# haoy945/DeMF

Hardware: AMD Instinct MI355X
Metric: DeMF fusion fwd+bwd scenes/sec at 20k pts + 530x730 RGB (higher is better)
Workload: dtype f32; 1 GPU; BASELINE configs[2]: full DeMF fusion hot path fwd+loss+bwd+allreduce+AdamW, 8 scenes/GPU x (20000 pts, 800x1120 -> 4-level 256-ch pyramid), 256 queries, H=8 L=4 P=2, fp32; compute_mode=f32, scenes_per_gpu=8, parallelism=dp1, cloud=uniform

## Files before the change

demf_amd/csrc/mlp.hip:

```cpp
#include "mlp_dev.h"
#include <type_traits>

namespace demf {

#ifdef DEMF_MLP_PROFILE
__device__ long long g_mlp_prof[16];
#define MP_T(k) const long long mp##k = __builtin_readcyclecounter();
#define MP_ACC(i, a, b) if (mp_on) mp_acc[i] += (b) - (a);
#else
#define MP_T(k)
#define MP_ACC(i, a, b)
#endif

template <int NT, int RT, int PRO, bool STATS, bool POOL = false, bool FIRST = false, bool RED = false,
          int CM = 0, bool SEL = false>
__global__ __launch_bounds__(256, 2) void mlp_gemm_kernel(MlpArgs p) {
  static_assert(!SEL || POOL, "SEL is a mode of the pooled epilogue");
  static_assert(!(STATS && RED) && !(FIRST && RED), "one column-sum epilogue at a time");
  constexpr bool BF16 = CM == 1, X3 = CM == 2;
  constexpr int LDB = X3 ? MLP_LD3 : MLP_LD;
  constexpr int WROWS = 32 * RT;
  constexpr int BROWS = 4 * WROWS;
  constexpr int NVEC = PRO == PRO_NONE ? 0 : (PRO == PRO_BNRELU ? 2 : 5);
  __shared__ __attribute__((aligned(16))) float s_a[4][WROWS * MLP_LD];
  __shared__ __attribute__((aligned(16))) float s_b[NT * 32 * LDB];
  __shared__ __attribute__((aligned(16))) float s_vec[NVEC ? NVEC * MLP_MAXK : 4];
  __shared__ float s_red[(STATS || RED) ? 4 * NT * 32 * 2 : (FIRST ? 4 * NT * 32 * 10 + 16 : 1)];
  __shared__ float4 s_pool[(POOL && RT == 1) ? 4 * NT * 32 : 1];
  if constexpr (NVEC > 0) {
    for (int i = threadIdx.x; i < NVEC * p.K; i += 256) s_vec[i] = p.vec[i];
    __syncthreads();
  }
  const int lane = threadIdx.x & 63;
  const int wave = threadIdx.x >> 6;
  const int lr = lane & 31, lh = lane >> 5;
  float* sa = s_a[wave];
  int bx = blockIdx.x, gx = gridDim.x, by = blockIdx.y;
  if constexpr (POOL) {
    if (p.halves == 2) {
      by = (bx >> 3) & 1;
      bx = (bx & 7) | ((bx >> 4) << 3);
      gx >>= 1;
    }
  }
  const int cofs = by * NT * 32;
  const int ntiles = (p.R + BROWS - 1) / BROWS;
  const int ksteps = (p.K + MLP_BK - 1) / MLP_BK;
  __shared__ int s_next;
  const bool dyn = p.sched != nullptr;
  const int grp = (bx >> 3) & (SCHED_GROUPS - 1);
  const int grp_first = gx / SCHED_GROUPS;
  auto group_tile = [&](int j) { return (((j >> 3) * SCHED_GROUPS + grp) << 3) + (j & 7); };
  int claimed = 0;
  float cs1[NT], cs2[NT];
#pragma unroll
  for (int nt = 0; nt < NT; ++nt) cs1[nt] = cs2[nt] = 0.f;
  float fs[FIRST ? NT : 1][10];
  float4 fcx = make_float4(0.f, 0.f, 0.f, 0.f);
  if constexpr (FIRST) {
#pragma unroll
    for (int nt = 0; nt < NT; ++nt)
#pragma unroll
      for (int q = 0; q < 10; ++q) fs[nt][q] = 0.f;
  }
  f32x16 acc[RT][NT];
  unsigned selbits = 0;
  if constexpr (SEL) {
#pragma unroll
    for (int nt = 0; nt < NT; ++nt) {
      const int col = cofs + nt * 32 + lr;
      if (col < p.N && p.fin.gamma[col] < 0.f) selbits |= 1u << nt;
    }
  }

  const int pr = lane >> 3, pc = (lane & 7) * 4;
  const int br = threadIdx.x >> 3;
  MlpRaw<PRO> pre[4 * RT];
  bool pok[4 * RT];
  float4 preb[NT];
  auto prefetch = [&](int tile, int ks) {
    const int k0 = ks * MLP_BK;
    const int row0 = tile * BROWS + wave * WROWS;
#pragma unroll
    for (int it = 0; it < 4 * RT; ++it) {
      const int row = row0 + it * 8 + pr, col = k0 + pc;
      pok[it] = row < p.R && col < p.K;
      mlp_fetch<PRO>(p, row, col, pok[it], pre[it]);
    }
#pragma unroll
    for (int i = 0; i < NT; ++i) {
      const int n = cofs + br + 32 * i, col = k0 + pc;
      preb[i] = make_float4(0.f, 0.f, 0.f, 0.f);
      if (p.ldb > 0) {
        const int kk = k0 + br, nn = cofs + 32 * i + pc;
        if (kk < p.K && nn < p.N) preb[i] = *reinterpret_cast<const float4*>(p.Bt + (size_t)kk * p.ldb + nn);
      } else if (n < p.N && col < p.K) {
        preb[i] = *reinterpret_cast<const float4*>(p.Bt + (size_t)n * p.K + col);
      }
    }
  };
#ifdef DEMF_MLP_PROFILE
  long long mp_acc[8] = {0, 0, 0, 0, 0, 0, 0, 0};
  const bool mp_on = blockIdx.x == 0 && blockIdx.y == 0 && threadIdx.x == 0;
#endif
  int tile = bx;
  if (tile < ntiles) prefetch(tile, 0);

  int ks = 0;
  while (tile < ntiles) {
    MP_T(0)
    const int k0 = ks * MLP_BK;
    const int row0 = tile * BROWS + wave * WROWS;
    const bool last_ks = ks == ksteps - 1;
    if (dyn && threadIdx.x == 0) {
      if (ks == 0) claimed = group_tile(grp_first + atomicAdd(p.sched + grp, 1));
      if (last_ks) s_next = claimed;
    }
    float* sb = s_b;
    if (ks == 0) {
#pragma unroll
      for (int rt = 0; rt < RT; ++rt)
#pragma unroll
        for (int nt = 0; nt < NT; ++nt)
#pragma unroll
          for (int r = 0; r < 16; ++r) acc[rt][nt][r] = 0.f;
    }
    lds_barrier();
    MP_T(1) MP_ACC(0, mp0, mp1)
    if constexpr (BF16) {
      char* sab = reinterpret_cast<char*>(sa);
      char* sbb = reinterpret_cast<char*>(sb);
#pragma unroll
      for (int it = 0; it < 4 * RT; ++it)
        *reinterpret_cast<bf16x4*>(sab + (it * 8 + pr) * (4 * MLP_LD) + 2 * pc) =
            to_bf16x4(mlp_xform<PRO>(p, s_vec, k0 + pc, pok[it], pre[it]));
#pragma unroll
      for (int i = 0; i < NT; ++i)
        if (p.ldb > 0) {
          char* d = sbb + (32 * i + pc) * (4 * MLP_LD) + 2 * br;
          *reinterpret_cast<__bf16*>(d) = (__bf16)preb[i].x;
          *reinterpret_cast<__bf16*>(d + 4 * MLP_LD) = (__bf16)preb[i].y;
          *reinterpret_cast<__bf16*>(d + 8 * MLP_LD) = (__bf16)preb[i].z;
          *reinterpret_cast<__bf16*>(d + 12 * MLP_LD) = (__bf16)preb[i].w;
        } else {
          *reinterpret_cast<bf16x4*>(sbb + (br + 32 * i) * (4 * MLP_LD) + 2 * pc) = to_bf16x4(preb[i]);
        }
    } else if constexpr (X3) {
#pragma unroll
      for (int it = 0; it < 4 * RT; ++it)
        *reinterpret_cast<float4*>(sa + (it * 8 + pr) * MLP_LD + pc) =
            mlp_xform<PRO>(p, s_vec, k0 + pc, pok[it], pre[it]);
      char* sbb = reinterpret_cast<char*>(sb);
#pragma unroll
      for (int i = 0; i < NT; ++i) {
        bf16x4 h, m, l;
        split3(preb[i], h, m, l);
        if (p.ldb > 0) {
#pragma unroll
          for (int e = 0; e < 4; ++e) {
            char* d = sbb + (32 * i + pc + e) * (4 * MLP_LD3) + 2 * br;
            *reinterpret_cast<__bf16*>(d) = h[e];
            *reinterpret_cast<__bf16*>(d + 64) = m[e];
            *reinterpret_cast<__bf16*>(d + 128) = l[e];
          }
        } else {
          char* d = sbb + (br + 32 * i) * (4 * MLP_LD3) + 2 * pc;
          *reinterpret_cast<bf16x4*>(d) = h;
          *reinterpret_cast<bf16x4*>(d + 64) = m;
          *reinterpret_cast<bf16x4*>(d + 128) = l;
        }
      }
    } else {
#pragma unroll
    for (int it = 0; it < 4 * RT; ++it)
      *reinterpret_cast<float4*>(sa + (it * 8 + pr) * MLP_LD + pc) =
          mlp_xform<PRO>(p, s_vec, k0 + pc, pok[it], pre[it]);
#pragma unroll
    for (int i = 0; i < NT; ++i)
      if (p.ldb > 0) {
        float* d = sb + (32 * i + pc) * MLP_LD + br;
        d[0] = preb[i].x; d[MLP_LD] = preb[i].y; d[2 * MLP_LD] = preb[i].z; d[3 * MLP_LD] = preb[i].w;
      } else {
        *reinterpret_cast<float4*>(sb + (br + 32 * i) * MLP_LD + pc) = preb[i];
      }
    }
    MP_T(2) MP_ACC(1, mp1, mp2)
    lds_barrier();
    MP_T(3) MP_ACC(2, mp2, mp3)
    constexpr bool DEFER = (POOL && RT == 2) || FIRST;
    const bool defer_prefetch = DEFER && last_ks;
    const int next_tile = last_ks ? (dyn ? s_next : tile + gx) : tile;
    const int next_ks = last_ks ? 0 : ks + 1;
    if (next_tile < ntiles && !defer_prefetch) prefetch(next_tile, next_ks);
    MP_T(4) MP_ACC(3, mp3, mp4)
    float4 yq[(FIRST || RED) ? 2 * RT * 2 : 1];
    float4 xq = make_float4(0.f, 0.f, 0.f, 0.f);
    auto first_load = [&](int half) {
#pragma unroll
      for (int j = 0; j < 2 * RT * 2; ++j) {
        const int id = lane + 64 * j;
        const int row = row0 + (id >> 3);
        yq[j] = make_float4(0.f, 0.f, 0.f, 0.f);
        if (row < p.R && cofs + 32 * half + 4 * (id & 7) < p.N)
          yq[j] = *reinterpret_cast<const float4*>(p.fY + (size_t)row * p.fld + p.fc0 + cofs + 32 * half + 4 * (id & 7));
      }
    };
    auto first_store = [&]() {
#pragma unroll
      for (int j = 0; j < 2 * RT * 2; ++j) {
        const int id = lane + 64 * j;
        *reinterpret_cast<float4*>(sa + (id >> 3) * MLP_LD + 4 * (id & 7)) = yq[j];
      }
    };
    if constexpr (RED) {
      if (last_ks) first_load(0);
    }
    if constexpr (FIRST) {
      if (last_ks) {
        first_load(0);
        if (lane < WROWS && row0 + lane < p.R)
          xq = *reinterpret_cast<const float4*>(p.fX + (size_t)(row0 + lane) * 4);
      }
    }
    if constexpr (BF16) {
      const char* sab = reinterpret_cast<const char*>(sa);
      const char* sbb = reinterpret_cast<const char*>(sb);
      const int kch = min(MLP_BK / 16, (p.K - k0 + 15) / 16);
      for (int c16 = 0; c16 < kch; ++c16) {
        bf16x8 a8[RT];
#pragma unroll
        for (int rt = 0; rt < RT; ++rt)
          a8[rt] = *reinterpret_cast<const bf16x8*>(sab + (rt * 32 + lr) * (4 * MLP_LD) + 2 * (c16 * 16 + 8 * lh));
#pragma unroll
        for (int nt = 0; nt < NT; ++nt) {
          const bf16x8 b8 = *reinterpret_cast<const bf16x8*>(sbb + (nt * 32 + lr) * (4 * MLP_LD) + 2 * (c16 * 16 + 8 * lh));
#pragma unroll
          for (int rt = 0; rt < RT; ++rt)
            acc[rt][nt] = __builtin_amdgcn_mfma_f32_32x32x16_bf16(a8[rt], b8, acc[rt][nt], 0, 0, 0);
        }
      }
    } else if constexpr (X3) {
      const char* sbb = reinterpret_cast<const char*>(sb);
      const int kch = min(MLP_BK / 16, (p.K - k0 + 15) / 16);
      for (int c16 = 0; c16 < kch; ++c16) {
        bf16x8 ah[RT], am[RT], al[RT];
#pragma unroll
        for (int rt = 0; rt < RT; ++rt) {
          const float* src = sa + (rt * 32 + lr) * MLP_LD + c16 * 16 + 8 * lh;
          split3(*reinterpret_cast<const float4*>(src), *reinterpret_cast<const float4*>(src + 4),
                 ah[rt], am[rt], al[rt]);
        }
#pragma unroll
        for (int nt = 0; nt < NT; ++nt) {
          const char* src = sbb + (nt * 32 + lr) * (4 * MLP_LD3) + 2 * (c16 * 16 + 8 * lh);
          const bf16x8 bh = *reinterpret_cast<const bf16x8*>(src);
          const bf16x8 bm = *reinterpret_cast<const bf16x8*>(src + 64);
          const bf16x8 bl = *reinterpret_cast<const bf16x8*>(src + 128);
#pragma unroll
          for (int rt = 0; rt < RT; ++rt) {
            acc[rt][nt] = __builtin_amdgcn_mfma_f32_32x32x16_bf16(al[rt], bh, acc[rt][nt], 0, 0, 0);
            acc[rt][nt] = __builtin_amdgcn_mfma_f32_32x32x16_bf16(ah[rt], bl, acc[rt][nt], 0, 0, 0);
            acc[rt][nt] = __builtin_amdgcn_mfma_f32_32x32x16_bf16(am[rt], bm, acc[rt][nt], 0, 0, 0);
            acc[rt][nt] = __builtin_amdgcn_mfma_f32_32x32x16_bf16(am[rt], bh, acc[rt][nt], 0, 0, 0);
            acc[rt][nt] = __builtin_amdgcn_mfma_f32_32x32x16_bf16(ah[rt], bm, acc[rt][nt], 0, 0, 0);
            acc[rt][nt] = __builtin_amdgcn_mfma_f32_32x32x16_bf16(ah[rt], bh, acc[rt][nt], 0, 0, 0);
          }
        }
      }
    } else {
    const int kchunks = min(MLP_BK / 8, (p.K - k0 + 7) / 8);
    for (int c8 = 0; c8 < kchunks; ++c8) {
      float4 a4[RT];
#pragma unroll
      for (int rt = 0; rt < RT; ++rt)
        a4[rt] = *reinterpret_cast<const float4*>(sa + (rt * 32 + lr) * MLP_LD + c8 * 8 + 4 * lh);
#pragma unroll
      for (int nt = 0; nt < NT; ++nt) {
        const float4 b4 = *reinterpret_cast<const float4*>(sb + (nt * 32 + lr) * MLP_LD + c8 * 8 + 4 * lh);
#pragma unroll
        for (int rt = 0; rt < RT; ++rt) {
          acc[rt][nt] = __builtin_amdgcn_mfma_f32_32x32x2f32(a4[rt].x, b4.x, acc[rt][nt], 0, 0, 0);
          acc[rt][nt] = __builtin_amdgcn_mfma_f32_32x32x2f32(a4[rt].y, b4.y, acc[rt][nt], 0, 0, 0);
          acc[rt][nt] = __builtin_amdgcn_mfma_f32_32x32x2f32(a4[rt].z, b4.z, acc[rt][nt], 0, 0, 0);
          acc[rt][nt] = __builtin_amdgcn_mfma_f32_32x32x2f32(a4[rt].w, b4.w, acc[rt][nt], 0, 0, 0);
        }
      }
    }
    }
    MP_T(5) MP_ACC(4, mp4, mp5)
    if (last_ks) {
#pragma unroll
      for (int nt = 0; nt < NT; ++nt) {
        float s1 = 0.f, s2 = 0.f;
        if constexpr (FIRST) {
          const int col = cofs + nt * 32 + lr;
          const bool cok = col < p.N;
          const float sc0 = cok ? p.fss[p.fc0 + col] : 0.f, sh0 = cok ? p.fss[p.fld + p.fc0 + col] : 0.f;
          const float mu0 = cok ? p.fmi[p.fc0 + col] : 0.f, is0 = cok ? p.fmi[p.fld + p.fc0 + col] : 0.f;
          first_store();
          if (nt == 0 && lane < WROWS) *reinterpret_cast<float4*>(sa + lane * MLP_LD + MLP_BK) = xq;
          if (nt + 1 < NT) first_load(nt + 1);
#pragma unroll
          for (int rt = 0; rt < RT; ++rt)
#pragma unroll
            for (int r = 0; r < 16; ++r) {
              const int rl = rt * 32 + (r & 3) + 8 * (r >> 2) + 4 * lh;
              if ((r & 3) == 0) __builtin_amdgcn_sched_barrier(0);
              if (row0 + rl < p.R && cok) {
                const float y = sa[rl * MLP_LD + lr];
                const float4 x = *reinterpret_cast<const float4*>(sa + rl * MLP_LD + MLP_BK);
                const float dz = __builtin_fmaf(y, sc0, sh0) > 0.f ? acc[rt][nt][r] : 0.f;
                fs[nt][0] += dz;
                fs[nt][1] = __builtin_fmaf(dz, (y - mu0) * is0, fs[nt][1]);
                fs[nt][2] = __builtin_fmaf(dz, x.x, fs[nt][2]);
                fs[nt][3] = __builtin_fmaf(dz, x.y, fs[nt][3]);
                fs[nt][4] = __builtin_fmaf(dz, x.z, fs[nt][4]);
                fs[nt][5] = __builtin_fmaf(dz, x.w, fs[nt][5]);
                fs[nt][6] = __builtin_fmaf(y, x.x, fs[nt][6]);
                fs[nt][7] = __builtin_fmaf(y, x.y, fs[nt][7]);
                fs[nt][8] = __builtin_fmaf(y, x.z, fs[nt][8]);
                fs[nt][9] = __builtin_fmaf(y, x.w, fs[nt][9]);
                if (nt == 0 && lr == 0 && by == 0) { fcx.x += x.x; fcx.y += x.y; fcx.z += x.z; fcx.w += x.w; }
              }
            }
        } else {
        float sc0 = 0.f, sh0 = 0.f, mu0 = 0.f, is0 = 0.f;
        if constexpr (RED) {
          const int col = cofs + nt * 32 + lr;
          if (col < p.N) {
            sc0 = p.fss[p.fc0 + col]; sh0 = p.fss[p.fld + p.fc0 + col];
            mu0 = p.fmi[p.fc0 + col]; is0 = p.fmi[p.fld + p.fc0 + col];
          }
          first_store();
          if (nt + 1 < NT) first_load(nt + 1);
        }
        auto store_tile = [&](auto full_c) {
          constexpr bool FULL = decltype(full_c)::value;
#pragma unroll
          for (int rt = 0; rt < RT; ++rt)
#pragma unroll
            for (int r = 0; r < 16; ++r) {
              const int row = row0 + rt * 32 + (r & 3) + 8 * (r >> 2) + 4 * lh;
              const float v = acc[rt][nt][r];
              const bool ok = FULL || (row < p.R && cofs + nt * 32 + lr < p.N);
              if (ok) p.Y[(size_t)row * p.ldy + cofs + nt * 32 + lr] = v;
              if constexpr (RED) {
                if ((r & 3) == 0) __builtin_amdgcn_sched_barrier(0);
                if (ok) {
                  const float y = sa[(rt * 32 + (r & 3) + 8 * (r >> 2) + 4 * lh) * MLP_LD + lr];
                  const float dz = __builtin_fmaf(y, sc0, sh0) > 0.f ? v : 0.f;
                  s1 += dz;
                  s2 = __builtin_fmaf(dz, (y - mu0) * is0, s2);
                }
              }
            }
          if constexpr (STATS) {
            using f32x2 = float __attribute__((ext_vector_type(2)));
            f32x2 a1 = {0.f, 0.f}, a2 = {0.f, 0.f};
#pragma unroll
            for (int rt = 0; rt < RT; ++rt)
#pragma unroll
              for (int r = 0; r < 16; r += 2) {
                const f32x2 v = {acc[rt][nt][r], acc[rt][nt][r + 1]};
                a1 += v;
                a2 = __builtin_elementwise_fma(v, v, a2);
              }
            s1 += a1.x + a1.y;
            s2 += a2.x + a2.y;
          }
        };
        if constexpr (POOL) {
          if (tile * BROWS + BROWS <= p.R && cofs + NT * 32 <= p.N) store_tile(std::true_type{});
          else store_tile(std::false_type{});
        } else {
#pragma unroll
          for (int rt = 0; rt < RT; ++rt)
#pragma unroll
            for (int r = 0; r < 16; ++r) {
              const int row = row0 + rt * 32 + (r & 3) + 8 * (r >> 2) + 4 * lh;
              const float v = acc[rt][nt][r];
              if (row < p.R && cofs + nt * 32 + lr < p.N)
                p.Y[(size_t)row * p.ldy + cofs + nt * 32 + lr] = v;
              if constexpr (RED) {
                if ((r & 3) == 0) __builtin_amdgcn_sched_barrier(0);
                if (row < p.R && cofs + nt * 32 + lr < p.N) {
                  const float y = sa[(rt * 32 + (r & 3) + 8 * (r >> 2) + 4 * lh) * MLP_LD + lr];
                  const float dz = __builtin_fmaf(y, sc0, sh0) > 0.f ? v : 0.f;
                  s1 += dz;
                  s2 = __builtin_fmaf(dz, (y - mu0) * is0, s2);
                }
              }
              if constexpr (STATS) {
                s1 += v;
                s2 = __builtin_fmaf(v, v, s2);
              }
            }
        }
        }
        cs1[nt] += s1;
        cs2[nt] += s2;
        if constexpr (POOL) {
          {
            const int col = cofs + nt * 32 + lr;
            if constexpr (SEL) {
              const unsigned flip = ((selbits >> nt) & 1u) << 31;
              if (p.ns == 16) pool_epilogue_sel<RT, NT, 16>(p, acc, nt, row0, col, lh, flip);
              else if (p.ns == 32) pool_epilogue_sel<RT, NT, 32>(p, acc, nt, row0, col, lh, flip);
              else if constexpr (RT == 2) pool_epilogue_sel<RT, NT, 64>(p, acc, nt, row0, col, lh, flip);
              else pool_half_reduce_sel<NT>(acc, nt, wave, lr, lh, s_pool, flip);
            } else {
            if (p.ns == 16) pool_epilogue<RT, NT, 16>(p, acc, nt, row0, col, lh);
            else if (p.ns == 32) pool_epilogue<RT, NT, 32>(p, acc, nt, row0, col, lh);
            else if constexpr (RT == 2) pool_epilogue<RT, NT, 64>(p, acc, nt, row0, col, lh);
            else pool_half_reduce<NT>(acc, nt, wave, lr, lh, s_pool);
            }
          }
        }
      }
      if constexpr (POOL && RT == 1) {
        if (p.ns == 64) {
          lds_barrier();
          if ((wave & 1) == 0 && lh == 0) {
            const int grow = row0;
#pragma unroll
            for (int nt = 0; nt < NT; ++nt) {
              const int col = cofs + nt * 32 + lr;
              if constexpr (SEL) {
                const float2* sp = reinterpret_cast<const float2*>(s_pool);
                const float2 a = sp[(wave * NT + nt) * 32 + lr];
                const float2 b = sp[((wave + 1) * NT + nt) * 32 + lr];
                const bool take_b = b.x > a.x;
                if (grow < p.R && col < p.N) {
                  const unsigned flip = ((selbits >> nt) & 1u) << 31;
                  const size_t o = (size_t)(grow / 64) * p.N + col;
                  p.pmax[o] = flip_sign(take_b ? b.x : a.x, flip);
                  p.amax[o] = __builtin_bit_cast(int, take_b ? b.y : a.y);
                }
                continue;
              }
              const float4 a = s_pool[(wave * NT + nt) * 32 + lr];
              const float4 b = s_pool[((wave + 1) * NT + nt) * 32 + lr];
              float mx = a.x, mn = a.y;
              int ax = __builtin_bit_cast(int, a.z), an = __builtin_bit_cast(int, a.w);
              if (b.x > mx) { mx = b.x; ax = __builtin_bit_cast(int, b.z); }
              if (b.y < mn) { mn = b.y; an = __builtin_bit_cast(int, b.w); }
              if (grow < p.R && col < p.N) {
                const size_t o = (size_t)(grow / 64) * p.N + col;
                p.pmax[o] = mx; p.pmin[o] = mn; p.amax[o] = ax; p.amin[o] = an;
              }
            }
          }
        }
      }
      if constexpr ((POOL && RT == 2) || FIRST) {
        if (next_tile < ntiles) prefetch(next_tile, next_ks);
      }
    }
    MP_T(6) MP_ACC(5, mp5, mp6)
    tile = next_tile;
    ks = next_ks;
  }
#ifdef DEMF_MLP_PROFILE
  if (mp_on) { for (int i = 0; i < 8; ++i) atomicAdd((unsigned long long*)&g_mlp_prof[i], (unsigned long long)mp_acc[i]); atomicAdd((unsigned long long*)&g_mlp_prof[15], 1ull); }
#endif
  if (dyn) {
    if (threadIdx.x == 0) {
      int* gdone = p.sched + SCHED_GROUPS;
      const int members = (int)(gridDim.x * gridDim.y) / SCHED_GROUPS;
      if (atomicAdd(gdone + 1 + grp, 1) == members - 1) {
        atomicExch(gdone + 1 + grp, 0);
        atomicExch(p.sched + grp, 0);
        if (atomicAdd(gdone, 1) == SCHED_GROUPS - 1) atomicExch(gdone, 0);
      }
    }
  }
  if constexpr (FIRST) {
#pragma unroll
    for (int nt = 0; nt < NT; ++nt)
#pragma unroll
      for (int q = 0; q < 10; ++q) {
        const float v = fs[nt][q] + __shfl_xor(fs[nt][q], 32);
        if (lh == 0) s_red[((wave * NT + nt) * 10 + q) * 32 + lr] = v;
      }
    fcx.x += __shfl_xor(fcx.x, 32); fcx.y += __shfl_xor(fcx.y, 32);
    fcx.z += __shfl_xor(fcx.z, 32); fcx.w += __shfl_xor(fcx.w, 32);
    if (lane == 0) {
      float* c = s_red + 4 * NT * 32 * 10 + wave * 4;
      c[0] = fcx.x; c[1] = fcx.y; c[2] = fcx.z; c[3] = fcx.w;
    }
    __syncthreads();
    constexpr int PER = NT * 10 * 32;
    for (int i = threadIdx.x; i < PER; i += 256) {
      const float v = s_red[i] + s_red[PER + i] + s_red[2 * PER + i] + s_red[3 * PER + i];
      const int nt = i / 320, q = (i / 32) % 10, c = i & 31;
      const int col = cofs + nt * 32 + c;
      if (col < p.N) {
        const int dst = q < 2 ? q * p.N + col : (q < 6 ? 2 * p.N + col * 4 + (q - 2) : 6 * p.N + col * 4 + (q - 6));
        atomicAdd(p.fsum + dst, (double)v);
      }
    }
    if (threadIdx.x < 4 && by == 0) {
      const float* c = s_red + 4 * NT * 32 * 10;
      atomicAdd(p.fsum + 10 * p.N + threadIdx.x,
                (double)(c[threadIdx.x] + c[4 + threadIdx.x] + c[8 + threadIdx.x] + c[12 + threadIdx.x]));
    }
  }
  if constexpr (STATS || RED) {
#pragma unroll
    for (int nt = 0; nt < NT; ++nt) {
      cs1[nt] += __shfl_xor(cs1[nt], 32);
      cs2[nt] += __shfl_xor(cs2[nt], 32);
      if (lh == 0) {
        s_red[(wave * NT + nt) * 64 + lr] = cs1[nt];
        s_red[(wave * NT + nt) * 64 + 32 + lr] = cs2[nt];
      }
    }
    __syncthreads();
    const int lin_s = (int)(blockIdx.y * gridDim.x + blockIdx.x);
    double* sdst = p.stats;
    if constexpr (RED) {
      if (p.vfin.ticket != nullptr && p.vfin.racc != nullptr) sdst = repl_copy(p.vfin.racc, p.fld, lin_s);
    } else {
      if (p.fin.ss != nullptr && p.fin.racc != nullptr) sdst = repl_copy(p.fin.racc, p.N, lin_s);
    }
    for (int i = threadIdx.x; i < NT * 64; i += 256) {
      const float v = s_red[i] + s_red[NT * 64 + i] + s_red[2 * NT * 64 + i] + s_red[3 * NT * 64 + i];
      const int nt = i >> 6, which = (i >> 5) & 1, c = i & 31;
      if (cofs + nt * 32 + c < p.N)
        atomicAdd(sdst + which * (RED ? p.fld : p.N) + (RED ? p.fc0 : 0) + cofs + nt * 32 + c, (double)v);
    }
  }
  if constexpr (RED) {
    if (p.vfin.ticket != nullptr) {
      sync_drained();
      if (threadIdx.x == 0)
        s_next = last_workgroup(p.vfin.ticket, (int)(gridDim.x * gridDim.y), (int)(blockIdx.y * gridDim.x + blockIdx.x));
      __syncthreads();
      if (s_next) bn_vec_finalize(p.vfin, p.fld, p.fc0, p.N, p.stats, threadIdx.x, 256);
    }
  }
  if constexpr (STATS) {
    if (p.fin.ss != nullptr) {
      sync_drained();
      if (threadIdx.x == 0) {
        const int total = (int)(gridDim.x * gridDim.y);
        const int lin = (int)(blockIdx.y * gridDim.x + blockIdx.x);
        const int ngroups = total < SCHED_GROUPS ? total : SCHED_GROUPS;
        const int g = lin % SCHED_GROUPS;
        const int members = total / SCHED_GROUPS + (g < total % SCHED_GROUPS ? 1 : 0);
        int* t = p.fin.ticket + FIN_OFF;
        int last = 0;
        asm volatile("s_waitcnt vmcnt(0)" ::: "memory");
        if (atomicAdd(t + 1 + g, 1) == members - 1) {
          atomicExch(t + 1 + g, 0);
          if (atomicAdd(t, 1) == ngroups - 1) { atomicExch(t, 0); last = 1; }
        }
        s_next = last;
      }
      __syncthreads();
      if (s_next) {
        const BnFin& f = p.fin;
        if (threadIdx.x == 0 && f.nbt != nullptr) *f.nbt += 1;
        for (int c = threadIdx.x; c < p.N; c += 256) {
          double s1 = __builtin_bit_cast(
              double, atomicExch(reinterpret_cast<unsigned long long*>(p.stats + c), 0ull));
          double s2 = __builtin_bit_cast(
              double, atomicExch(reinterpret_cast<unsigned long long*>(p.stats + p.N + c), 0ull));
          if (f.racc != nullptr) { s1 += repl_take(f.racc, p.N, c); s2 += repl_take(f.racc, p.N, p.N + c); }
          bn_finalize_channel(c, p.N, f.count, s1, s2, f.gamma, f.beta, f.eps, f.momentum, f.rmean,
                              f.rvar, f.ss, f.mi, f.conv_bias);
        }
      }
    }
  }
}

static int mlp_grid(int R, int brows) {
  const int tiles = (R + brows - 1) / brows;
  const int cap = sw().gemm_grid;
  return tiles < cap ? (tiles > 0 ? tiles : 1) : cap;
}

template <int PRO, bool STATS, bool POOL, bool RED, int CM>
static int launch_gemm_t(const MlpArgs& a, hipStream_t s);

template <int PRO, bool STATS, bool POOL = false, bool RED = false>
static int launch_gemm(const MlpArgs& a, hipStream_t s) {
  switch (compute_mode()) {
    case 1: return launch_gemm_t<PRO, STATS, POOL, RED, 1>(a, s);
    case 2: {
      if (sw().x3_mask & (PRO >= PRO_DY_DENSE ? 2 : 1)) return launch_gemm_t<PRO, STATS, POOL, RED, 2>(a, s);
      return launch_gemm_t<PRO, STATS, POOL, RED, 0>(a, s);
    }
    default: return launch_gemm_t<PRO, STATS, POOL, RED, 0>(a, s);
  }
}

template <int PRO, bool STATS, bool POOL, bool RED, int BF16>
static int launch_gemm_t(const MlpArgs& a, hipStream_t s) {
  if constexpr ((BF16 == 1 || BF16 == 2) && !RED && STATS && PRO == PRO_BNRELU) {
    if (fwd_pc_takes(a, POOL)) {
      const int rc = launch_fwd_pc(a, BF16, POOL, s);
      if (rc == DEMF_OK) set_last_form(DEMF_FORM_PC);
      return rc;
    }
    if (fwd_res_takes(a, POOL)) {
      const int rc = launch_fwd_res(a, BF16, POOL, s);
      if (rc == DEMF_OK) set_last_form(DEMF_FORM_RES);
      return rc;
    }
  }
  if (a.st != 0) {
    set_error("mlp_gemm: bf16 row storage (st=%d) is only built into the weight-resident forward (K = 64, "
              "N = 64 / 128, R >= 16384, bf16 compute mode)", a.st);
    return DEMF_EUNSUPPORTED;
  }
  if constexpr ((BF16 == 1 || BF16 == 2) && !POOL && !STATS && (PRO == PRO_DY_DENSE || PRO == PRO_DY_SPARSE)) {
    constexpr bool SP = PRO == PRO_DY_SPARSE;
    if (dx_tile_takes(a, SP, RED)) {
      const int rc = launch_dx_tile(a, BF16, SP, RED, s);
      if (rc != LAUNCH_TRY_NEXT) { set_last_form(DEMF_FORM_TILE); return rc; }
    }
  }
  if constexpr ((BF16 == 1 || BF16 == 2) && !RED && !POOL && STATS && (PRO == PRO_BNRELU || PRO == PRO_NONE)) {
    if (fwd_tile_takes(a, PRO == PRO_BNRELU)) {
      const int rc = launch_fwd_tile(a, BF16, PRO == PRO_BNRELU, s);
      if (rc != LAUNCH_TRY_NEXT) { set_last_form(DEMF_FORM_TILE); return rc; }
    }
  }
  set_last_form(DEMF_FORM_GENERIC);
  const dim3 block(256);
  constexpr int RT2_MAX = PRO >= PRO_DY_DENSE ? 2 : 4;
  constexpr int NT_MAX = PRO >= PRO_DY_DENSE ? 4 : 8;
  const int nt = (a.N + 31) / 32;
  if (nt < 1 || nt > (POOL ? NT_MAX : 16)) {
    set_error("mlp_gemm: N=%d unsupported for this prologue (max %d columns per launch)", a.N,
              (POOL ? NT_MAX : 16) * 32);
    return DEMF_EUNSUPPORTED;
  }
  if constexpr (POOL) {
    const bool half64 = a.ns == 64 && nt <= 4 && !sw().pool_halves;
    const bool rt2 = a.ns == 64 && !half64;
    const int ntl = rt2 ? (nt < 2 ? nt : 2) : (nt < 4 ? nt : 4);
    const int ys = (nt + ntl - 1) / ntl;
    int gx = mlp_grid(a.R, rt2 ? 256 : 128);
    MlpArgs a2 = a;
    dim3 grid(gx, ys);
    if (ys == 2) {
      gx = ((gx + 7) / 8) * 8;
      a2.halves = 2;
      grid = dim3(2 * gx, 1);
    }
    {
      const int brows = rt2 ? 256 : 128;
      const int tiles = (a.R + brows - 1) / brows;
      if (sw().pool_dyn && ys == 1 && tiles > gx && a.K > MLP_BK && gx % (8 * SCHED_GROUPS) == 0)
        a2.sched = sched_slot();
    }
    const bool sel = a.pmin == nullptr && a.fin.gamma != nullptr;
#define PGO(NTv, RTv)                                                                                       \
    do {                                                                                                    \
      if (sel) hipLaunchKernelGGL((mlp_gemm_kernel<NTv, RTv, PRO, STATS, true, false, false, BF16, true>), grid, block, 0, s, a2); \
      else hipLaunchKernelGGL((mlp_gemm_kernel<NTv, RTv, PRO, STATS, true, false, false, BF16>), grid, block, 0, s, a2);           \
    } while (0)
    if (rt2) { if (ntl == 1) PGO(1, 2); else PGO(2, 2); }
    else if (ntl == 1) PGO(1, 1);
    else if (ntl == 2) PGO(2, 1);
    else if (ntl == 3) PGO(3, 1);
    else PGO(4, 1);
#undef PGO
    return check_launch("mlp_gemm_pool");
  } else {
  const int tiles1 = (a.R + 127) / 128;
  if ((tiles1 < 192 && nt > 1) || nt > NT_MAX || (BF16 == 2 && nt > 4 && sw().x3_wide_split)) {
    int ysplit = (sw().split_target + tiles1 - 1) / tiles1;
    if (ysplit < (nt + 3) / 4) ysplit = (nt + 3) / 4;
    if (ysplit > nt) ysplit = nt;
    const int ntl = (nt + ysplit - 1) / ysplit;
    const dim3 grid(tiles1, (nt + ntl - 1) / ntl);
    switch (ntl) {
#define SPLIT(NTv)                                                                              \
      case NTv: hipLaunchKernelGGL((mlp_gemm_kernel<NTv, 1, PRO, STATS, POOL, false, RED, BF16>), grid, block, 0, s, a); break;
      SPLIT(1) SPLIT(2) SPLIT(3) SPLIT(4)
#undef SPLIT
      default: break;
    }
    if (ntl <= 4) return check_launch("mlp_gemm");
  }
#define GO(NTv, RTv)                                                                            \
  do {                                                                                          \
    MlpArgs a3 = a;                                                                             \
    const int gxv = mlp_grid(a.R, 128 * RTv);                                                   \
    const int tilesv = (a.R + 128 * RTv - 1) / (128 * RTv);                                     \
    if (tilesv > gxv && a.K > MLP_BK && gxv % (8 * SCHED_GROUPS) == 0) a3.sched = sched_slot();                                \
    hipLaunchKernelGGL((mlp_gemm_kernel<NTv, RTv, PRO, STATS, POOL, false, RED, BF16>), dim3(gxv), block, 0, s, a3); \
  } while (0)
#define CASE(NTv)                                                                               \
  case NTv:                                                                                     \
    if constexpr (NTv <= NT_MAX && (BF16 != 2 || NTv <= 4)) {                                   \
      if constexpr (NTv <= RT2_MAX && !RED) GO(NTv, 2); else GO(NTv, 1);                        \
    }                                                                                           \
    break;
  if constexpr (BF16 == 2) {
    if (nt > 4) return launch_gemm_t<PRO, STATS, POOL, RED, 0>(a, s);
  }
  switch (nt) {
    CASE(1) CASE(2) CASE(3) CASE(4) CASE(5) CASE(6) CASE(7) CASE(8)
  }
#undef CASE
#undef GO
  return check_launch("mlp_gemm");
  }
}

static int mlp_check(int R, int K, int N, int ldx) {
  DEMF_REQUIRE(R >= 0 && K >= 4 && K % 4 == 0 && K <= MLP_MAXK && N >= 1 && N <= 256 && ldx >= K &&
                   ldx % 4 == 0,
               "mlp: bad sizes R=%d K=%d N=%d ldx=%d (K%%4==0, K<=512, 1<=N<=256)", R, K, N, ldx);
  return DEMF_OK;
}

}

using namespace demf;


extern "C" int demf_mlp_gemm_fwd(int R, int K, int N, int ldx, const float* X,
                                 const float* pro_scale_shift, const float* Wt, float* Y,
                                 double* stats, demf_stream_t stream) {
  if (int e = mlp_check(R, K, N, ldx)) return e;
  if (R == 0) return DEMF_OK;
  DEMF_REQUIRE(X && Wt && Y, "mlp_gemm_fwd: null pointer");
  MlpArgs a{};
  a.R = R; a.K = K; a.N = N; a.ldx = ldx; a.ldy = N; a.X = X; a.vec = pro_scale_shift; a.Bt = Wt;
  a.Y = Y; a.stats = stats;
  hipStream_t s = (hipStream_t)stream;
  if (pro_scale_shift)
    return stats ? launch_gemm<PRO_BNRELU, true>(a, s) : launch_gemm<PRO_BNRELU, false>(a, s);
  return stats ? launch_gemm<PRO_NONE, true>(a, s) : launch_gemm<PRO_NONE, false>(a, s);
}

extern "C" int demf_mlp_gemm_fwd_pool(int R, int K, int N, int ldx, const float* X,
                                      const float* pro_scale_shift, const float* Wt, float* Y,
                                      double* stats, int ns, float* pmax, float* pmin, int* amax,
                                      int* amin, demf_stream_t stream) {
  if (int e = mlp_check(R, K, N, ldx)) return e;
  const bool ok = (ns == 16 || ns == 32 || ns == 64) && R % ns == 0;
  if (!ok) {
    set_error("mlp_gemm_fwd_pool: ns=%d with R=%d N=%d is not fused", ns, R, N);
    return DEMF_EUNSUPPORTED;
  }
  if (R == 0) return DEMF_OK;
  DEMF_REQUIRE(X && Wt && Y && pro_scale_shift && stats && pmax && pmin && amax && amin,
               "mlp_gemm_fwd_pool: null pointer");
  MlpArgs a{};
  a.R = R; a.K = K; a.N = N; a.ldx = ldx; a.ldy = N; a.X = X; a.vec = pro_scale_shift; a.Bt = Wt;
  a.Y = Y; a.stats = stats; a.ns = ns; a.pmax = pmax; a.pmin = pmin; a.amax = amax; a.amin = amin;
  return launch_gemm<PRO_BNRELU, true, true>(a, (hipStream_t)stream);
}

template <typename Launch>
static int launch_with_finalize(MlpArgs& a, BnFin fin, Launch launch, hipStream_t s) {
  fin.ticket = sw().no_fin ? nullptr : sched_slot();
  fin.racc = fin.ticket != nullptr && a.N <= ACC_MAX_N && sw().acc_repl_fwd ? accum_slot() : nullptr;
  a.fin = fin;
  if (fin.ticket != nullptr) return launch(a);
  a.fin.ss = nullptr;
  if (int e = launch(a)) return e;
  return launch_bn_finalize(a.N, a.stats, fin, s);
}

static int fin_check(long long count, const float* gamma, const float* beta, const float* ss,
                     const float* mi, const double* stats) {
  DEMF_REQUIRE(count >= 1 && gamma && beta && ss && mi && stats, "mlp_gemm_fwd_bn: bad BN arguments");
  return DEMF_OK;
}

static int mlp_gemm_fwd_bn_impl(int R, int K, int N, int ldx, const float* X,
                                const float* pro_scale_shift, const float* Wt, float* Y,
                                double* stats, const float* gamma, const float* beta, float eps,
                                float momentum, float* running_mean, float* running_var,
                                long long* num_batches_tracked, float* scale_shift,
                                float* mean_invstd, const float* conv_bias, int st, demf_stream_t stream) {
  if (int e = mlp_check(R, K, N, ldx)) return e;
  DEMF_REQUIRE(R >= 1 && X && Wt && Y, "mlp_gemm_fwd_bn: null pointer / no rows");
  if (int e = fin_check(R, gamma, beta, scale_shift, mean_invstd, stats)) return e;
  MlpArgs a{};
  a.R = R; a.K = K; a.N = N; a.ldx = ldx; a.ldy = N; a.X = X; a.vec = pro_scale_shift; a.Bt = Wt;
  a.Y = Y; a.stats = stats; a.st = st;
  hipStream_t s = (hipStream_t)stream;
  BnFin fin{(double)R, gamma, beta, conv_bias, eps, momentum, running_mean, running_var,
            num_batches_tracked, scale_shift, mean_invstd, nullptr};
  if (pro_scale_shift)
    return launch_with_finalize(a, fin, [s](const MlpArgs& b) { return launch_gemm<PRO_BNRELU, true>(b, s); }, s);
  return launch_with_finalize(a, fin, [s](const MlpArgs& b) { return launch_gemm<PRO_NONE, true>(b, s); }, s);
}

extern "C" int demf_mlp_gemm_fwd_bn(int R, int K, int N, int ldx, const float* X,
                                    const float* pro_scale_shift, const float* Wt, float* Y,
                                    double* stats, const float* gamma, const float* beta, float eps,
                                    float momentum, float* running_mean, float* running_var,
                                    long long* num_batches_tracked, float* scale_shift,
                                    float* mean_invstd, const float* conv_bias, demf_stream_t stream) {
  return mlp_gemm_fwd_bn_impl(R, K, N, ldx, X, pro_scale_shift, Wt, Y, stats, gamma, beta, eps, momentum,
                              running_mean, running_var, num_batches_tracked, scale_shift, mean_invstd,
                              conv_bias, 0, stream);
}

extern "C" int demf_mlp_gemm_fwd_bn_st(int R, int K, int N, int ldx, const void* X,
                                       const float* pro_scale_shift, const float* Wt, void* Y,
                                       double* stats, const float* gamma, const float* beta, float eps,
                                       float momentum, float* running_mean, float* running_var,
                                       long long* num_batches_tracked, float* scale_shift,
                                       float* mean_invstd, const float* conv_bias, int store_flags,
                                       demf_stream_t stream) {
  DEMF_REQUIRE(store_flags >= 1 && store_flags <= 3 && pro_scale_shift, "mlp_gemm_fwd_bn_st: store_flags in 1..3, BN prologue");
  return mlp_gemm_fwd_bn_impl(R, K, N, ldx, (const float*)X, pro_scale_shift, Wt, (float*)Y, stats, gamma, beta,
                              eps, momentum, running_mean, running_var, num_batches_tracked, scale_shift,
                              mean_invstd, conv_bias, store_flags, stream);
}

static int mlp_gemm_fwd_pool_bn_impl(int R, int K, int N, int ldx, const float* X,
                                     const float* pro_scale_shift, const float* Wt, float* Y,
                                     double* stats, int ns, float* pmax, float* pmin, int* amax,
                                     int* amin, const float* gamma, const float* beta, float eps,
                                     float momentum, float* running_mean, float* running_var,
                                     long long* num_batches_tracked, float* scale_shift,
                                     float* mean_invstd, const float* conv_bias, int st,
                                     demf_stream_t stream) {
  if (int e = mlp_check(R, K, N, ldx)) return e;
  const bool ok = (ns == 16 || ns == 32 || ns == 64) && R % ns == 0 && R >= 1;
  if (!ok) {
    set_error("mlp_gemm_fwd_pool_bn: ns=%d with R=%d N=%d is not fused", ns, R, N);
    return DEMF_EUNSUPPORTED;
  }
  DEMF_REQUIRE(X && Wt && (Y || st == 4) && pro_scale_shift && pmax && amax && (pmin == nullptr) == (amin == nullptr),
               "mlp_gemm_fwd_pool_bn: null pointer");
  if (int e = fin_check(R, gamma, beta, scale_shift, mean_invstd, stats)) return e;
  MlpArgs a{};
  a.R = R; a.K = K; a.N = N; a.ldx = ldx; a.ldy = N; a.X = X; a.vec = pro_scale_shift; a.Bt = Wt;
  a.Y = Y; a.stats = stats; a.ns = ns; a.pmax = pmax; a.pmin = pmin; a.amax = amax; a.amin = amin;
  a.st = st;
  hipStream_t s = (hipStream_t)stream;
  BnFin fin{(double)R, gamma, beta, conv_bias, eps, momentum, running_mean, running_var,
            num_batches_tracked, scale_shift, mean_invstd, nullptr};
  return launch_with_finalize(a, fin, [s](const MlpArgs& b) { return launch_gemm<PRO_BNRELU, true, true>(b, s); }, s);
}

extern "C" int demf_mlp_gemm_fwd_pool_bn(int R, int K, int N, int ldx, const float* X,
                                         const float* pro_scale_shift, const float* Wt, float* Y,
                                         double* stats, int ns, float* pmax, float* pmin, int* amax,
                                         int* amin, const float* gamma, const float* beta, float eps,
                                         float momentum, float* running_mean, float* running_var,
                                         long long* num_batches_tracked, float* scale_shift,
                                         float* mean_invstd, const float* conv_bias,
                                         demf_stream_t stream) {
  return mlp_gemm_fwd_pool_bn_impl(R, K, N, ldx, X, pro_scale_shift, Wt, Y, stats, ns, pmax, pmin, amax, amin,
                                   gamma, beta, eps, momentum, running_mean, running_var,
                                   num_batches_tracked, scale_shift, mean_invstd, conv_bias, 0, stream);
}

extern "C" int demf_mlp_gemm_fwd_pool_bn_st(int R, int K, int N, int ldx, const void* X,
                                            const float* pro_scale_shift, const float* Wt, void* Y,
                                            double* stats, int ns, float* pmax, int* amax,
                                            const float* gamma, const float* beta, float eps,
                                            float momentum, float* running_mean, float* running_var,
                                            long long* num_batches_tracked, float* scale_shift,
                                            float* mean_invstd, const float* conv_bias, int store_flags,
                                            demf_stream_t stream) {
  DEMF_REQUIRE(store_flags >= 1 && store_flags <= 4, "mlp_gemm_fwd_pool_bn_st: store_flags in 1..4");
  return mlp_gemm_fwd_pool_bn_impl(R, K, N, ldx, (const float*)X, pro_scale_shift, Wt, (float*)Y, stats, ns,
                                   pmax, nullptr, amax, nullptr, gamma, beta, eps, momentum, running_mean,
                                   running_var, num_batches_tracked, scale_shift, mean_invstd, conv_bias,
                                   store_flags, stream);
}

__global__ __launch_bounds__(256) void mlp_first_stats_k(int R, int N0, const float* __restrict__ X,
                                                         const float* __restrict__ W0, double* __restrict__ mom,
                                                         BnFin fin, int bf16) {
  float m[14];
#pragma unroll
  for (int i = 0; i < 14; ++i) m[i] = 0.f;
  double acc[14];
#pragma unroll
  for (int i = 0; i < 14; ++i) acc[i] = 0.0;
  int n = 0;
  for (int r = blockIdx.x * 256 + threadIdx.x; r < R; r += gridDim.x * 256) {
    float4 x = *reinterpret_cast<const float4*>(X + (size_t)r * 4);
    if (bf16) { x.x = (float)(__bf16)x.x; x.y = (float)(__bf16)x.y; x.z = (float)(__bf16)x.z; x.w = (float)(__bf16)x.w; }
    const float v[4] = {x.x, x.y, x.z, x.w};
    int t = 4;
#pragma unroll
    for (int i = 0; i < 4; ++i) {
      m[i] += v[i];
#pragma unroll
      for (int j = i; j < 4; ++j) { m[t] = __builtin_fmaf(v[i], v[j], m[t]); ++t; }
    }
    if (++n == 64) {
#pragma unroll
      for (int i = 0; i < 14; ++i) { acc[i] += (double)m[i]; m[i] = 0.f; }
      n = 0;
    }
  }
#pragma unroll
  for (int i = 0; i < 14; ++i) acc[i] += (double)m[i];
  __shared__ double s_m[4][14];
  __shared__ int s_last;
#pragma unroll
  for (int i = 0; i < 14; ++i) {
    double v = acc[i];
    for (int d = 32; d >= 1; d >>= 1) v += __shfl_xor(v, d);
    if ((threadIdx.x & 63) == 0) s_m[threadIdx.x >> 6][i] = v;
  }
  __syncthreads();
  if (threadIdx.x < 14)
    atomicAdd(mom + threadIdx.x, (s_m[0][threadIdx.x] + s_m[1][threadIdx.x]) + (s_m[2][threadIdx.x] + s_m[3][threadIdx.x]));
  sync_drained();
  if (threadIdx.x == 0) s_last = last_workgroup(fin.ticket, (int)gridDim.x, (int)blockIdx.x);
  __syncthreads();
  if (!s_last) return;
  __shared__ double s_t[14];
  if (threadIdx.x < 14)
    s_t[threadIdx.x] = __builtin_bit_cast(double, atomicExch(reinterpret_cast<unsigned long long*>(mom + threadIdx.x), 0ull));
  __syncthreads();
  if (threadIdx.x == 0 && fin.nbt != nullptr) *fin.nbt += 1;
  for (int c = threadIdx.x; c < N0; c += 256) {
    double w[4];
#pragma unroll
    for (int k = 0; k < 4; ++k) {
      const float wk = W0[c * 4 + k];
      w[k] = bf16 ? (double)(float)(__bf16)wk : (double)wk;
    }
    double s1 = 0.0, s2 = 0.0;
    int t = 4;
#pragma unroll
    for (int i = 0; i < 4; ++i) {
      s1 += w[i] * s_t[i];
#pragma unroll
      for (int j = i; j < 4; ++j) { s2 += (i == j ? 1.0 : 2.0) * w[i] * w[j] * s_t[t]; ++t; }
    }
    bn_finalize_channel(c, N0, fin.count, s1, s2, fin.gamma, fin.beta, fin.eps, fin.momentum, fin.rmean, fin.rvar,
                        fin.ss, fin.mi, fin.conv_bias);
  }
}

extern "C" int demf_mlp_first_stats(int R, int N0, const float* X, const float* W0, double* moments,
                                    const float* gamma, const float* beta, float eps, float momentum,
                                    float* running_mean, float* running_var, long long* num_batches_tracked,
                                    float* scale_shift, float* mean_invstd, const float* conv_bias,
                                    demf_stream_t stream) {
  DEMF_REQUIRE(R >= 1 && N0 >= 1 && X && W0 && moments, "mlp_first_stats: bad arguments");
  if (int e = fin_check(R, gamma, beta, scale_shift, mean_invstd, moments)) return e;
  BnFin fin{(double)R, gamma, beta, conv_bias, eps, momentum, running_mean, running_var,
            num_batches_tracked, scale_shift, mean_invstd, sched_slot()};
  DEMF_REQUIRE(fin.ticket != nullptr, "mlp_first_stats: needs the counter ring (DEMF_STATIC_TILES=1 is set)");
  int grid = cdiv(R, 256 * 16);
  if (grid > 256) grid = 256;
  if (grid < 1) grid = 1;
  hipLaunchKernelGGL(mlp_first_stats_k, dim3(grid), dim3(256), 0, (hipStream_t)stream, R, N0, X, W0, moments, fin,
                     compute_mode() == 1 ? 1 : 0);
  return check_launch("mlp_first_stats");
}

extern "C" int demf_mlp_gemm_fwd_bn_x4(int R, int N, const float* X4, const float* W0,
                                       const float* prev_scale_shift, const float* Wt, float* Y, double* stats,
                                       const float* gamma, const float* beta, float eps, float momentum,
                                       float* running_mean, float* running_var, long long* num_batches_tracked,
                                       float* scale_shift, float* mean_invstd, const float* conv_bias,
                                       demf_stream_t stream) {
  const int cm = compute_mode();
  DEMF_REQUIRE((cm == 1 || cm == 2) && N == 64 && R >= 64 * 256 && X4 && W0 && prev_scale_shift && Wt && Y,
               "mlp_gemm_fwd_bn_x4: unsupported shape / mode R=%d N=%d mode=%d (or null pointer)", R, N, cm);
  if (int e = fin_check(R, gamma, beta, scale_shift, mean_invstd, stats)) return e;
  MlpArgs a{};
  a.R = R; a.K = 64; a.N = N; a.ldx = 4; a.ldy = N; a.X = X4; a.W0 = W0; a.vec = prev_scale_shift; a.Bt = Wt;
  a.Y = Y; a.stats = stats; a.st = 8;
  hipStream_t s = (hipStream_t)stream;
  BnFin fin{(double)R, gamma, beta, conv_bias, eps, momentum, running_mean, running_var,
            num_batches_tracked, scale_shift, mean_invstd, nullptr};
  return launch_with_finalize(a, fin, [s](const MlpArgs& b) { return launch_gemm<PRO_BNRELU, true>(b, s); }, s);
}

struct DxReduce {
  const float* Yprev;
  const float* ss;
  const float* mi;
  double* g12;
  const float* gamma = nullptr;
  float* vec6 = nullptr;
  float* dgamma = nullptr;
  float* dbeta = nullptr;
};

static int mlp_bwd_dx_impl(bool w_direct, int R, int N, int K, int ldo, const float* G, const float* dP,
                           const int* arg, int ns, const float* Y, const float* vec6,
                           const float* Wtt, float* dX, const DxReduce* red, demf_stream_t stream) {
  DEMF_REQUIRE(R >= 0 && N >= 4 && N % 4 == 0 && K >= 1 && ldo >= K,
               "mlp_gemm_bwd_dx: bad sizes R=%d N=%d K=%d ldo=%d", R, N, K, ldo);
  if (R == 0) return DEMF_OK;
  DEMF_REQUIRE(Y && vec6 && Wtt && dX && (G || (dP && arg && ns >= 1)), "mlp_gemm_bwd_dx: null pointer");
  hipStream_t s = (hipStream_t)stream;
  const int cstep = (!sw().dx_chunks && K <= 512) ? K : 128;
  for (int c0 = 0; c0 < K; c0 += cstep) {
    MlpArgs a{};
    a.R = R; a.K = N; a.N = (K - c0) < cstep ? (K - c0) : cstep; a.ldx = N; a.ldy = ldo; a.X = Y;
    a.G = G; a.dP = dP; a.arg = arg; a.ns = ns; a.vec = vec6;
    if (w_direct) { a.Bt = Wtt + c0; a.ldb = K; }
    else a.Bt = Wtt + (size_t)c0 * N;
    a.Y = dX + c0; a.stats = nullptr;
    int e;
    if (red) {
      a.fY = red->Yprev; a.fss = red->ss; a.fmi = red->mi; a.stats = red->g12; a.fld = K; a.fc0 = c0;
      if (red->gamma != nullptr)
        a.vfin = BnVecFin{(double)R, red->gamma, red->ss, red->mi, red->vec6, red->dgamma, red->dbeta, sched_slot(),
                          nullptr};
      if (a.vfin.ticket != nullptr && K <= ACC_MAX_N && sw().acc_repl_red) a.vfin.racc = accum_slot();
      e = G ? launch_gemm<PRO_DY_DENSE, false, false, true>(a, s)
            : launch_gemm<PRO_DY_SPARSE, false, false, true>(a, s);
    } else {
      e = G ? launch_gemm<PRO_DY_DENSE, false>(a, s) : launch_gemm<PRO_DY_SPARSE, false>(a, s);
    }
    if (e) return e;
  }
  if (red && red->gamma != nullptr && sw().static_tiles)
    return demf_bn_bwd_vectors(K, (long long)R, red->g12, red->gamma, red->ss, red->mi, red->vec6, red->dgamma,
                               red->dbeta, stream);
  return DEMF_OK;
}

extern "C" int demf_mlp_gemm_bwd_dx(int R, int N, int K, int ldo, const float* G, const float* dP,
                                    const int* arg, int ns, const float* Y, const float* vec6,
                                    const float* Wtt, float* dX, demf_stream_t stream) {
  return mlp_bwd_dx_impl(false, R, N, K, ldo, G, dP, arg, ns, Y, vec6, Wtt, dX, nullptr, stream);
}

extern "C" int demf_mlp_gemm_bwd_dx_w(int R, int N, int K, int ldo, const float* G, const float* dP,
                                      const int* arg, int ns, const float* Y, const float* vec6,
                                      const float* W, float* dX, demf_stream_t stream) {
  return mlp_bwd_dx_impl(true, R, N, K, ldo, G, dP, arg, ns, Y, vec6, W, dX, nullptr, stream);
}

extern "C" int demf_mlp_gemm_bwd_dx_red(int R, int N, int K, int ldo, const float* G, const float* dP,
                                        const int* arg, int ns, const float* Y, const float* vec6,
                                        const float* W, float* dX, const float* Yprev,
                                        const float* scale_shift_prev, const float* mean_invstd_prev,
                                        double* g12_prev, demf_stream_t stream) {
  DEMF_REQUIRE(K % 4 == 0 && Yprev && scale_shift_prev && mean_invstd_prev && g12_prev,
               "mlp_gemm_bwd_dx_red: bad arguments (K %% 4 == 0)");
  const DxReduce red{Yprev, scale_shift_prev, mean_invstd_prev, g12_prev};
  return mlp_bwd_dx_impl(true, R, N, K, ldo, G, dP, arg, ns, Y, vec6, W, dX, &red, stream);
}

extern "C" int demf_mlp_gemm_bwd_dx_red_v(int R, int N, int K, int ldo, const float* G, const float* dP,
                                          const int* arg, int ns, const float* Y, const float* vec6,
                                          const float* W, float* dX, const float* Yprev,
                                          const float* scale_shift_prev, const float* mean_invstd_prev,
                                          double* g12_prev, const float* gamma_prev, float* vec6_prev,
                                          float* dgamma_prev, float* dbeta_prev, demf_stream_t stream) {
  DEMF_REQUIRE(K % 4 == 0 && Yprev && scale_shift_prev && mean_invstd_prev && g12_prev && gamma_prev &&
                   vec6_prev && dgamma_prev && dbeta_prev,
               "mlp_gemm_bwd_dx_red_v: bad arguments (K %% 4 == 0)");
  DxReduce red{Yprev, scale_shift_prev, mean_invstd_prev, g12_prev};
  red.gamma = gamma_prev; red.vec6 = vec6_prev; red.dgamma = dgamma_prev; red.dbeta = dbeta_prev;
  return mlp_bwd_dx_impl(true, R, N, K, ldo, G, dP, arg, ns, Y, vec6, W, dX, &red, stream);
}

__global__ void mlp_first_finish_k(int N, double count, double* __restrict__ sums,
                                   const float* __restrict__ gamma, const float* __restrict__ mi,
                                   float* __restrict__ dW, float* __restrict__ dgamma,
                                   float* __restrict__ dbeta) {
  __shared__ double s_cx[4];
  if (threadIdx.x < 4) s_cx[threadIdx.x] = sums[10 * N + threadIdx.x];
  __syncthreads();
  const int c = threadIdx.x;
  if (c < N) {
    const double g1 = sums[c], g2 = sums[N + c];
    const double mean = mi[c], is = mi[N + c];
    const double gi = (double)gamma[c] * is;
    const double a = -gi * is * (g2 / count);
    const double b = -gi * (g1 / count) - a * mean;
#pragma unroll
    for (int k = 0; k < 4; ++k) {
      dW[c * 4 + k] = (float)(gi * sums[2 * N + c * 4 + k] + a * sums[6 * N + c * 4 + k] + b * s_cx[k]);
      sums[2 * N + c * 4 + k] = 0.0;
      sums[6 * N + c * 4 + k] = 0.0;
    }
    sums[c] = 0.0;
    sums[N + c] = 0.0;
    dgamma[c] = (float)g2;
    dbeta[c] = (float)g1;
  }
  if (threadIdx.x < 4) sums[10 * N + threadIdx.x] = 0.0;
}

extern "C" int demf_mlp_gemm_bwd_dx_first(int R, int N, int K0, const float* G, const float* Y1,
                                          const float* vec6, const float* W1, const float* X0,
                                          const float* Y0, const float* ss0, const float* mi0,
                                          double* sums, demf_stream_t stream) {
  DEMF_REQUIRE(R >= 1 && N >= 4 && N % 4 == 0 && N <= MLP_MAXK && K0 >= 4 && K0 % 4 == 0 && K0 <= 64,
               "mlp_gemm_bwd_dx_first: bad sizes R=%d N=%d K0=%d (K0 <= 64)", R, N, K0);
  DEMF_REQUIRE(G && Y1 && vec6 && W1 && X0 && Y0 && ss0 && mi0 && sums,
               "mlp_gemm_bwd_dx_first: null pointer");
  hipStream_t s = (hipStream_t)stream;
  MlpArgs a{};
  a.R = R; a.K = N; a.N = K0; a.ldx = N; a.ldy = K0; a.X = Y1; a.G = G; a.vec = vec6;
  a.Bt = W1; a.ldb = K0; a.Y = nullptr; a.stats = nullptr;
  a.fX = X0; a.fY = Y0; a.fss = ss0; a.fmi = mi0; a.fsum = sums; a.fld = K0; a.fc0 = 0;
  const int gx = mlp_grid(R, 128);
  const int tiles = (R + 127) / 128;
  if (tiles > gx && a.K > MLP_BK && gx % (8 * SCHED_GROUPS) == 0) a.sched = sched_slot();
#define FIRSTGO(NTv, CMv) \
  hipLaunchKernelGGL((mlp_gemm_kernel<NTv, 1, PRO_DY_DENSE, false, false, true, false, CMv>), dim3(gx), dim3(256), 0, s, a)
  const int cm = compute_mode();
  if (K0 <= 32) {
    if (cm == 1) FIRSTGO(1, 1); else if (cm == 2) FIRSTGO(1, 2); else FIRSTGO(1, 0);
  } else {
    if (cm == 1) FIRSTGO(2, 1); else if (cm == 2) FIRSTGO(2, 2); else FIRSTGO(2, 0);
  }
#undef FIRSTGO
  return check_launch("mlp_gemm_bwd_dx_first");
}

extern "C" int demf_mlp_first_finish(int N0, long long count, double* sums, const float* gamma0,
                                     const float* mean_invstd0, float* dW0, float* dgamma0,
                                     float* dbeta0, demf_stream_t stream) {
  DEMF_REQUIRE(N0 >= 1 && N0 <= 64 && count >= 1 && sums && gamma0 && mean_invstd0 && dW0 && dgamma0 &&
                   dbeta0, "mlp_first_finish: bad arguments");
  hipLaunchKernelGGL(mlp_first_finish_k, dim3(1), dim3(64), 0, (hipStream_t)stream, N0, (double)count,
                     sums, gamma0, mean_invstd0, dW0, dgamma0, dbeta0);
  return check_launch("mlp_first_finish");
}

#ifdef DEMF_MLP_PROFILE
extern "C" int demf_mlp_prof_read(long long* out16, int reset) {
  if (hipMemcpyFromSymbol(out16, HIP_SYMBOL(demf::g_mlp_prof), 16 * sizeof(long long)) != hipSuccess) return -1;
  if (reset) {
    long long z[16] = {0};
    if (hipMemcpyToSymbol(HIP_SYMBOL(demf::g_mlp_prof), z, sizeof(z)) != hipSuccess) return -1;
  }
  return 0;
}
#endif
```

Measured before the change: 1932 scenes/s.

## Spread first-layer BN moment atomics over copies and batch row loads

```diff
diff --git a/demf_amd/csrc/mlp.hip b/demf_amd/csrc/mlp.hip
--- a/demf_amd/csrc/mlp.hip
+++ b/demf_amd/csrc/mlp.hip
@@ -875,6 +875,30 @@
                                    store_flags, stream);
 }
 
+constexpr int FS_ROWS = 16;
+constexpr int FS_COPIES = 32;
+constexpr int FS_PITCH = 16;
+constexpr int FS_TICKET = 14;
+static_assert(FS_COPIES * FS_PITCH <= ACC_SLOT_DOUBLES, "the copies fit one block of the accumulator ring");
+
+template <int CTRL, int ROW_MASK = 0xF>
+__device__ __forceinline__ double dpp_f64(double old, double v) {
+  const unsigned long long o = __builtin_bit_cast(unsigned long long, old), x = __builtin_bit_cast(unsigned long long, v);
+  const unsigned lo = (unsigned)__builtin_amdgcn_update_dpp((int)(unsigned)o, (int)(unsigned)x, CTRL, ROW_MASK, 0xF, false);
+  const unsigned hi =
+      (unsigned)__builtin_amdgcn_update_dpp((int)(unsigned)(o >> 32), (int)(unsigned)(x >> 32), CTRL, ROW_MASK, 0xF, false);
+  return __builtin_bit_cast(double, ((unsigned long long)hi << 32) | lo);
+}
+__device__ __forceinline__ double wave_sum_lane63(double v) {
+  v += dpp_f64<0xB1>(v, v);
+  v += dpp_f64<0x4E>(v, v);
+  v += dpp_f64<0x141>(v, v);
+  v += dpp_f64<0x140>(v, v);
+  v += dpp_f64<0x142, 0xA>(0.0, v);
+  v += dpp_f64<0x143, 0xC>(0.0, v);
+  return v;
+}
+
 __global__ __launch_bounds__(256) void mlp_first_stats_k(int R, int N0, const float* __restrict__ X,
                                                          const float* __restrict__ W0, double* __restrict__ mom,
                                                          BnFin fin, int bf16) {
@@ -884,22 +908,32 @@
   double acc[14];
 #pragma unroll
   for (int i = 0; i < 14; ++i) acc[i] = 0.0;
-  int n = 0;
-  for (int r = blockIdx.x * 256 + threadIdx.x; r < R; r += gridDim.x * 256) {
-    float4 x = *reinterpret_cast<const float4*>(X + (size_t)r * 4);
-    if (bf16) { x.x = (float)(__bf16)x.x; x.y = (float)(__bf16)x.y; x.z = (float)(__bf16)x.z; x.w = (float)(__bf16)x.w; }
-    const float v[4] = {x.x, x.y, x.z, x.w};
-    int t = 4;
-#pragma unroll
-    for (int i = 0; i < 4; ++i) {
-      m[i] += v[i];
-#pragma unroll
-      for (int j = i; j < 4; ++j) { m[t] = __builtin_fmaf(v[i], v[j], m[t]); ++t; }
-    }
-    if (++n == 64) {
+  const long long G = (long long)gridDim.x * 256;
+  int batches = 0;
+  for (long long r0 = (long long)blockIdx.x * 256 + threadIdx.x; r0 < R; r0 += FS_ROWS * G) {
+    float4 x[FS_ROWS];
+#pragma unroll
+    for (int u = 0; u < FS_ROWS; ++u) {
+      const long long r = r0 + u * G;
+      x[u] = r < R ? *reinterpret_cast<const float4*>(X + (size_t)r * 4) : make_float4(0.f, 0.f, 0.f, 0.f);
+    }
+#pragma unroll
+    for (int u = 0; u < FS_ROWS; ++u) {
+      float4 q = x[u];
+      if (bf16) { q.x = (float)(__bf16)q.x; q.y = (float)(__bf16)q.y; q.z = (float)(__bf16)q.z; q.w = (float)(__bf16)q.w; }
+      const float v[4] = {q.x, q.y, q.z, q.w};
+      int t = 4;
+#pragma unroll
+      for (int i = 0; i < 4; ++i) {
+        m[i] += v[i];
+#pragma unroll
+        for (int j = i; j < 4; ++j) { m[t] = __builtin_fmaf(v[i], v[j], m[t]); ++t; }
+      }
+    }
+    if (++batches == 64 / FS_ROWS) {
 #pragma unroll
       for (int i = 0; i < 14; ++i) { acc[i] += (double)m[i]; m[i] = 0.f; }
-      n = 0;
+      batches = 0;
     }
   }
 #pragma unroll
@@ -908,20 +942,49 @@
   __shared__ int s_last;
 #pragma unroll
   for (int i = 0; i < 14; ++i) {
-    double v = acc[i];
-    for (int d = 32; d >= 1; d >>= 1) v += __shfl_xor(v, d);
-    if ((threadIdx.x & 63) == 0) s_m[threadIdx.x >> 6][i] = v;
+    const double v = wave_sum_lane63(acc[i]);
+    if ((threadIdx.x & 63) == 63) s_m[threadIdx.x >> 6][i] = v;
   }
   __syncthreads();
+  const int total = (int)gridDim.x;
+  const int ncopies = total < FS_COPIES ? total : FS_COPIES;
+  const int copy = (int)blockIdx.x % FS_COPIES;
+  double* dst = fin.racc != nullptr ? fin.racc + copy * FS_PITCH : mom;
   if (threadIdx.x < 14)
-    atomicAdd(mom + threadIdx.x, (s_m[0][threadIdx.x] + s_m[1][threadIdx.x]) + (s_m[2][threadIdx.x] + s_m[3][threadIdx.x]));
+    atomicAdd(dst + threadIdx.x, (s_m[0][threadIdx.x] + s_m[1][threadIdx.x]) + (s_m[2][threadIdx.x] + s_m[3][threadIdx.x]));
   sync_drained();
-  if (threadIdx.x == 0) s_last = last_workgroup(fin.ticket, (int)gridDim.x, (int)blockIdx.x);
+  if (threadIdx.x == 0) {
+    if (fin.racc != nullptr) {
+      drain_vmem();
+      const int members = total / FS_COPIES + (copy < total % FS_COPIES ? 1 : 0);
+      unsigned* sub = reinterpret_cast<unsigned*>(dst + FS_TICKET);
+      int last = 0;
+      if (atomicAdd(sub, 1u) == (unsigned)(members - 1)) {
+        atomicExch(sub, 0u);
+        int* top = fin.ticket + BV_OFF;
+        if (atomicAdd(top, 1) == ncopies - 1) { atomicExch(top, 0); last = 1; }
+      }
+      s_last = last;
+    } else {
+      s_last = last_workgroup(fin.ticket, total, (int)blockIdx.x);
+    }
+  }
   __syncthreads();
   if (!s_last) return;
   __shared__ double s_t[14];
-  if (threadIdx.x < 14)
+  if (fin.racc != nullptr) {
+    __shared__ double s_c[FS_COPIES * 14];
+    for (int p = threadIdx.x; p < ncopies * 14; p += 256)
+      s_c[p] = __builtin_bit_cast(double, atomicExch(reinterpret_cast<unsigned long long*>(fin.racc + (p / 14) * FS_PITCH + p % 14), 0ull));
+    __syncthreads();
+    if (threadIdx.x < 14) {
+      double t = 0.0;
+      for (int r = 0; r < ncopies; ++r) t += s_c[r * 14 + threadIdx.x];
+      s_t[threadIdx.x] = t;
+    }
+  } else if (threadIdx.x < 14) {
     s_t[threadIdx.x] = __builtin_bit_cast(double, atomicExch(reinterpret_cast<unsigned long long*>(mom + threadIdx.x), 0ull));
+  }
   __syncthreads();
   if (threadIdx.x == 0 && fin.nbt != nullptr) *fin.nbt += 1;
   for (int c = threadIdx.x; c < N0; c += 256) {
@@ -954,6 +1017,7 @@
   BnFin fin{(double)R, gamma, beta, conv_bias, eps, momentum, running_mean, running_var,
             num_batches_tracked, scale_shift, mean_invstd, sched_slot()};
   DEMF_REQUIRE(fin.ticket != nullptr, "mlp_first_stats: needs the counter ring (DEMF_STATIC_TILES=1 is set)");
+  fin.racc = accum_slot();
   int grid = cdiv(R, 256 * 16);
   if (grid > 256) grid = 256;
   if (grid < 1) grid = 1;
```

Result: no change. 1929 scenes/s (-0.2%).
